# zhenyuw16/Uni3DETR

Hardware: AMD Instinct MI355X
Metric: scenes/sec (fwd+bwd) SUN-RGB-D 20k pts, 300 queries (higher is better)
Workload: dtype bf16

## Files before the change

### include/u3d_hip.h

```cpp
#ifndef U3D_HIP_H_
#define U3D_HIP_H_

#include <stddef.h>
#include <stdint.h>

#ifdef __cplusplus
extern "C" {
#endif

typedef struct ihipStream_t* u3d_stream;

enum {
  U3D_OK = 0,
  U3D_ERR_ARG = -1,
  U3D_ERR_UNSUPPORTED = -2,
  U3D_ERR_LAUNCH = -3,
  U3D_ERR_WORKSPACE = -4
};

enum { U3D_F32 = 0, U3D_BF16 = 1 };

int32_t u3d_version(void);
const char* u3d_strerror(int32_t code);

// ... 194 lines not shown
int32_t u3d_skinny_wgrad_batched(const void* const* dy, const void* const* x, float* const* partial, const int32_t* n, const int32_t* k,
                                 int32_t count, int32_t m, int32_t dy_skinny, u3d_stream s);

int64_t u3d_bn_stats_workspace(int32_t n_cap, int32_t c);
int32_t u3d_bn_stats(const void* x, const int32_t* n_dev, int32_t n_cap, int32_t c, int32_t dtype,
                     double* sums, void* workspace, int64_t workspace_bytes, u3d_stream s);
int32_t u3d_bn_finalize(const double* sums, const int32_t* n_dev, int32_t n_cap, int32_t c, float eps, float momentum,
                        float* running_mean, float* running_var, int64_t* num_batches, float* mean, float* invstd,
                        u3d_stream s);
int32_t u3d_bn_forward_stats(const void* x, const int32_t* n_dev, int32_t n_cap, int32_t c, int32_t dtype, float eps,
                             float momentum, float* running_mean, float* running_var, int64_t* num_batches, float* mean,
                             float* invstd, void* workspace, int64_t workspace_bytes, u3d_stream s);
int32_t u3d_bn_finalize_partials(const double* partial, int32_t nblocks, int32_t rows_per_block, const int32_t* n_dev,
                                 int32_t n_cap, int32_t c, float eps, float momentum, float* running_mean, float* running_var,
                                 int64_t* num_batches, float* mean, float* invstd, u3d_stream s);
int32_t u3d_bn_apply(const void* x, const float* mean, const float* invstd, const float* gamma,
                     const float* beta, const void* residual, int32_t relu, void* y, void* planes,
                     const int32_t* n_dev, int32_t n_cap, int32_t c, int32_t dtype, const int32_t* row_map, const void* post_add,
                     u3d_stream s);
int32_t u3d_bn_bwd_stats(const void* dy, const void* y, const void* x, const float* mean, const float* invstd,
                         const float* gamma, const float* beta, int32_t relu, const int32_t* n_dev, int32_t n_cap,
                         int32_t c, int32_t dtype, double* sums, void* workspace, int64_t workspace_bytes,
                         const int32_t* row_map, float* sums_f32, u3d_stream s);
int32_t u3d_bn_bwd_apply(const void* dy, const void* y, const void* x, const float* mean, const float* invstd,
                         const float* gamma, const float* beta, const double* sums, int32_t relu, void* dx, void* dres, void* planes,
                         const int32_t* n_dev, int32_t n_cap, int32_t c, int32_t dtype, const int32_t* row_map, u3d_stream s);
int32_t u3d_bn_apply_sum(const void* const* x, const float* const* mean, const float* const* invstd, const float* const* gamma,
                         const float* const* beta, const int32_t* const* idx, int32_t levels, void* out, const int32_t* n_dev,
                         int32_t n_cap, int32_t c, int32_t dtype, u3d_stream s);
int32_t u3d_bn_bwd_apply_sum(const void* dout, const void* const* x, const float* const* mean, const float* const* invstd,
                             const float* const* gamma, const float* const* beta, const double* const* sums,
                             const int32_t* const* idx, void* const* dx, int32_t levels, const int32_t* n_dev, int32_t n_cap,
                             int32_t c, int32_t dtype, u3d_stream s);

int32_t u3d_to_dense(const void* feat, const int32_t* coors, const int32_t* n_dev, int32_t n_cap, int32_t c,
                     void* dense, int32_t dz, int32_t dy, int32_t dx, int32_t dtype, u3d_stream s);
int32_t u3d_from_dense(const void* dense, const int32_t* coors, const int32_t* n_dev, int32_t n_cap, int32_t c,
                       void* feat, int32_t dz, int32_t dy, int32_t dx, int32_t dtype, u3d_stream s);

int32_t u3d_gather_rows(const void* in, const int32_t* idx, int32_t n, int32_t row_bytes, void* out, u3d_stream s);
int32_t u3d_scatter_rows(const void* in, const int32_t* idx, int32_t n, int32_t row_bytes, void* out, u3d_stream s);

int32_t u3d_fps(const float* base, const int64_t* set_off, const int32_t* set_n, int32_t nsets, int32_t max_n,
                int32_t m, int32_t* out_idx, float* temp, int64_t temp_stride, int32_t* err, int64_t poll_ticks, int32_t max_wg,
                u3d_stream s);
int32_t u3d_fps2(const float* base, const float* base2, int32_t split, const int64_t* set_off, const int32_t* set_n,
// ... 349 lines not shown
```

### uni3detr_amd/csrc/igemm_wgrad.hip

```cpp
#include "igemm_common.h"
#include "conv_in.h"

#ifndef WGRAD_DMA_SPREAD
#define WGRAD_DMA_SPREAD 1
#endif

template <int WAVES_M, int WAVES_N, int WM, int WN>
__global__ __launch_bounds__(WAVES_M* WAVES_N * 64) void k_igemm_wgrad(const u16* __restrict__ in, const u16* __restrict__ dout,
                                                                        const int* __restrict__ nbr, int ld, float* __restrict__ partial,
                                                                        const int* __restrict__ n_out_dev, int n_out_cap, int cin,
                                                                        int cout, int kvol, int co_blocks) {
  constexpr int NT = WAVES_M * WAVES_N * 64;
  constexpr int TM = WAVES_M * WM * 16, TN = WAVES_N * WN * 16, RK = 64;
  constexpr int LDA = TM + 16, LDD = TN + 16;
  constexpr int A_ELEMS = RK * LDA, D_ELEMS = RK * LDD;
  constexpr int A_SEGS = RK * TM / 8 / NT, D_SEGS = RK * TN / 8 / NT;
  static_assert(RK * TM / 8 % NT == 0 && RK * TN / 8 % NT == 0, "tile/thread mismatch");
  extern __shared__ __attribute__((aligned(16))) u16 smem[];
  constexpr int STAGE_ELEMS = A_ELEMS + D_ELEMS;

  const int n_out = min(*n_out_dev, n_out_cap);
  const int nsplit = gridDim.x, split = blockIdx.x, kap = blockIdx.y;
  const int ci0 = (blockIdx.z / co_blocks) * TM, co0 = (blockIdx.z % co_blocks) * TN;
  const int tid = threadIdx.x, lane = tid & 63, wv = tid >> 6;
// ... 580 lines not shown
    const f32x4 v6 = *(const f32x4*)(p + (long long)(k + 6) * stride), v7 = *(const f32x4*)(p + (long long)(k + 7) * stride);
    a += v0; b += v1; c += v2; d += v3; a += v4; b += v5; c += v6; d += v7;
  }
  for (; k < nsplit; ++k) a += *(const f32x4*)(p + (long long)k * stride);
  return (a + b) + (c + d);
}

struct WgradGroups { unsigned char mult[U3D_WGRAD_BATCH_MAX]; };
__global__ void k_wgrad_batch_reduce(WgradBatch bt, WgradGroups gr, const float* __restrict__ partial, long long n, int nsplit,
                                     long long partial_stride) {
  const int b = blockIdx.y;
  const int g = gr.mult[b];
  long long i = ((long long)blockIdx.x * blockDim.x + threadIdx.x) * 4;
  if (i >= n || g == 0) return;
  *(f32x4*)(bt.dw[b] + i) = wgrad_sum_splits(partial + (long long)b * partial_stride + i, n, nsplit * g);
}

__global__ void k_igemm_wgrad_reduce(const float* __restrict__ partial, float* __restrict__ dw, long long n, int nsplit) {
  long long i = ((long long)blockIdx.x * blockDim.x + threadIdx.x) * 4;
  if (i >= n) return;
  *(f32x4*)(dw + i) = wgrad_sum_splits(partial + i, n, nsplit);
}

__device__ __forceinline__ void wgrad_reduce_tile(const float* __restrict__ partial, long long n, int nsplit, int ca, int cb, int a,
                                                  int b0, int k0, int k1, float (&tile)[64][10]) {
  const int t = threadIdx.x, col = t & 63;
  for (int k = k0 + (t >> 6); k < k1; k += 4) {
    float s = 0.f;
    if (b0 + col < cb) {
      const float* p = partial + ((long long)k * ca + a) * cb + b0 + col;
      float acc[8];
#pragma unroll
      for (int j = 0; j < 8; ++j) acc[j] = 0.f;
      int sp = 0;
      for (; sp + 8 <= nsplit; sp += 8) {
#pragma unroll
        for (int j = 0; j < 8; ++j) acc[j] += p[(long long)(sp + j) * n];
      }
      for (; sp < nsplit; ++sp) acc[0] += p[(long long)sp * n];
      s = ((acc[0] + acc[1]) + (acc[2] + acc[3])) + ((acc[4] + acc[5]) + (acc[6] + acc[7]));
    }
    tile[col][k - k0] = s;
  }
  __syncthreads();
}
__global__ __launch_bounds__(256) void k_igemm_wgrad_reduce_oik(const float* __restrict__ partial, float* __restrict__ dw, long long n,
                                                                int nsplit, int kvol, int cin, int cout) {
  __shared__ float tile[64][10];
  const int ci = blockIdx.x, co0 = blockIdx.y * 64;
  const int kper = (kvol + gridDim.z - 1) / gridDim.z, k0 = blockIdx.z * kper, k1 = min(kvol, k0 + kper);
  wgrad_reduce_tile(partial, n, nsplit, cin, cout, ci, co0, k0, k1, tile);
  const int nk = k1 - k0;
  for (int idx = threadIdx.x; idx < 64 * nk; idx += 256) {
    const int cl = idx / nk, k = idx % nk;
    if (co0 + cl < cout) dw[((long long)(co0 + cl) * cin + ci) * kvol + k0 + k] = tile[cl][k];
  }
}
__global__ __launch_bounds__(256) void k_igemm_wgrad_reduce_abk(const float* __restrict__ partial, float* __restrict__ dw, long long n,
                                                                int nsplit, int kvol, int ca, int cb) {
  __shared__ float tile[64][10];
  const int a = blockIdx.x, b0 = blockIdx.y * 64;
  const int kper = (kvol + gridDim.z - 1) / gridDim.z, k0 = blockIdx.z * kper, k1 = min(kvol, k0 + kper);
  wgrad_reduce_tile(partial, n, nsplit, ca, cb, a, b0, k0, k1, tile);
  const int nk = k1 - k0;
  for (int idx = threadIdx.x; idx < 64 * nk; idx += 256) {
    const int cl = idx / nk, k = idx % nk;
    if (b0 + cl < cb) dw[((long long)a * cb + b0 + cl) * kvol + k0 + k] = tile[cl][k];
  }
}

typedef void (*wgrad_kernel_t)(const u16*, const u16*, const int*, int, float*, const int*, int, int, int, int, int);
typedef void (*wgrad_batch_kernel_t)(WgradBatch, float*, const int*, int, int, int, int, long long);
enum { WG_NONE, WG_CONVIN, WG_NARROW, WG_GLDS8_256, WG_GLDS_256, WG_GLDS_128, WG_GLDS_64, WG_REG_32, WG_REG_16, WG_COUNT };
struct WgradKernel {
  wgrad_kernel_t fn;
  wgrad_batch_kernel_t batch;
  int tile, threads;
  size_t lds;
};
static const WgradKernel WGRAD_KERNELS[WG_COUNT] = {
    {}, {}, {},
    {k_igemm_wgrad_glds8_256, nullptr, 256, 512, 4 * 64 * 256 * 2},
    {k_igemm_wgrad_glds_256, k_wgrad_batch_256, 256, 512, 4 * 64 * 256 * 2},
    {k_igemm_wgrad_glds_128, k_wgrad_batch_128, 128, 256, 4 * 64 * 128 * 2},
    {k_igemm_wgrad_glds_64, k_wgrad_batch_64, 64, 256, 4 * 64 * 64 * 2},
    {k_igemm_wgrad<2, 2, 1, 1>, nullptr, 32, 256, 4 * 64 * (32 + 16) * 2},
    {k_igemm_wgrad<1, 1, 1, 1>, nullptr, 16, 64, 4 * 64 * (16 + 16) * 2},
};
enum WgReduce { WG_RED_OWN, WG_RED_KIO, WG_RED_OIK, WG_RED_ABK };

struct WgradPlan {
// ... 88 lines not shown
  return U3D_OK;
}

static unsigned long long wgrad_lds_mask[WG_COUNT][2] = {};

extern "C" int32_t u3d_igemm_wgrad_bf16(const void* in, const void* dout, const int32_t* nbr, int32_t ld, float* dw,
                                        const int32_t* n_out_dev, int32_t n_out_cap, int32_t cin, int32_t cout, int32_t kvol,
                                        int32_t out_layout, void* workspace, int64_t workspace_bytes, u3d_stream s) {
  U3D_REQUIRE(in && dout && dw && n_out_dev && workspace && (nbr || kvol == 1), U3D_ERR_ARG);
  const WgradPlan p = wgrad_plan(n_out_cap, cin, cout, kvol, nbr != nullptr, out_layout);
  if (!p.served()) return U3D_ERR_UNSUPPORTED;
  if (p.family == WG_NARROW) {
    if (n_out_cap <= 0) { hipMemsetAsync(dw, 0, sizeof(float) * kvol * cin * cout, s); return U3D_OK; }
    return u3d_launch_wgrad_narrow(in, dout, nbr, ld, dw, n_out_dev, n_out_cap, cin, cout, kvol, out_layout, workspace, workspace_bytes, s);
  }
  U3D_REQUIRE(workspace_bytes >= p.workspace, U3D_ERR_WORKSPACE);
  if (p.family == WG_CONVIN) return u3d_launch_conv_in_wgrad(in, dout, nbr, ld, dw, n_out_dev, n_out_cap, kvol, (float*)workspace, s);
  const WgradKernel& k = WGRAD_KERNELS[p.family];
  if (p.lds > 64 * 1024) u3d_allow_lds_impl((const void*)k.fn, (int)p.lds, &wgrad_lds_mask[p.family][0]);
  hipLaunchKernelGGL(k.fn, p.grid, dim3(p.threads), p.lds, s, (const u16*)in, (const u16*)dout, nbr, ld, (float*)workspace, n_out_dev, n_out_cap,
                     cin, cout, kvol, p.co_blocks);
  if (hipGetLastError() != hipSuccess) return U3D_ERR_LAUNCH;
  const long long n = (long long)kvol * cin * cout;
  if (p.reduce == WG_RED_ABK)
    hipLaunchKernelGGL(k_igemm_wgrad_reduce_abk, dim3(cin, u3d_cdiv(cout, 64), kvol > 9 ? 3 : 1), dim3(256), 0, s, (const float*)workspace, dw, n, p.nsplit, kvol, cin, cout);
  else if (p.reduce == WG_RED_OIK)
    hipLaunchKernelGGL(k_igemm_wgrad_reduce_oik, dim3(cin, u3d_cdiv(cout, 64), kvol > 9 ? 3 : 1), dim3(256), 0, s, (const float*)workspace, dw, n, p.nsplit, kvol, cin, cout);
  else
    hipLaunchKernelGGL(k_igemm_wgrad_reduce, dim3(u3d_cdiv(n / 4, 256)), dim3(256), 0, s, (const float*)workspace, dw, n, p.nsplit);
  U3D_CHECK_LAUNCH();
  return U3D_OK;
}

static WgradPlan wgrad_plan_batched(int count, int n_rows, int cin, int cout) {
  const int mn = cin < cout ? cin : cout;
  int tile = (mn >= 256 && cin % 256 == 0 && cout % 256 == 0) ? 256 : ((mn >= 128 && cin % 128 == 0 && cout % 128 == 0) ? 128 : 64);
  const int ntiles = u3d_cdiv(n_rows > 0 ? n_rows : 1, 64);
  WgradPlan p;
  for (;;) {
    p.tile = tile;
    p.ci_blocks = u3d_cdiv(cin, tile);
    p.co_blocks = u3d_cdiv(cout, tile);
    const int per = (count > 0 ? count : 1) * p.ci_blocks * p.co_blocks;
    int ns = u3d_cdiv(768, per);
    int max_ns = ntiles / 8 > 0 ? ntiles / 8 : 1;
    if (ns > max_ns) ns = max_ns;
    if (ns < 1) ns = 1;
    p.nsplit = ns;
    if (tile == 64 || (long long)per * ns >= 192) break;
    tile /= 2;
// ... 34 lines not shown
```

### uni3detr_amd/csrc/rowops.hip

```cpp
#include "common.h"
#include <type_traits>

typedef unsigned short u16;
__device__ __forceinline__ float ld_elem(const float* p, long long i) { return p[i]; }
__device__ __forceinline__ float ld_elem(const u16* p, long long i) { return __uint_as_float(((unsigned)p[i]) << 16); }
__device__ __forceinline__ void st_elem(float* p, long long i, float v) { p[i] = v; }
__device__ __forceinline__ void st_elem(u16* p, long long i, float v) {
  unsigned u = __float_as_uint(v);
  if ((u & 0x7fffffffu) > 0x7f800000u) { p[i] = (u16)((u >> 16) | 0x40u); return; }
  u += 0x7fffu + ((u >> 16) & 1u);
  p[i] = (u16)(u >> 16);
}

static inline int st_rows_per_block(int n_cap, int c) {
  if (n_cap >= 131072) return c >= 128 ? 256 : 512;
  return n_cap >= 32768 ? 128 : 16;
}

template <typename T> struct VecOf;
template <> struct VecOf<float> { static constexpr int N = 4; };
template <> struct VecOf<u16> { static constexpr int N = 8; };

template <typename T>
__device__ __forceinline__ void load_vec(const T* p, float* out);
// ... 8 lines not shown
  unsigned w[4] = {v.x, v.y, v.z, v.w};
#pragma unroll
  for (int i = 0; i < 4; ++i) { out[2 * i] = __uint_as_float(w[i] << 16); out[2 * i + 1] = __uint_as_float(w[i] & 0xffff0000u); }
}

static inline bool al16(const void* p) { return ((uintptr_t)p & 15) == 0; }
template <int V>
__device__ __forceinline__ void load_cols(const float* __restrict__ p, int col0, float* out) {
#pragma unroll
  for (int i = 0; i < V; i += 4) {
    const float4 t = *(const float4*)(p + col0 + i);
    out[i] = t.x; out[i + 1] = t.y; out[i + 2] = t.z; out[i + 3] = t.w;
  }
}
template <int V>
__device__ __forceinline__ void load_cols_d(const double* __restrict__ p, int col0, float scale, float* out) {
#pragma unroll
  for (int i = 0; i < V; i += 2) {
    const double2 t = *(const double2*)(p + col0 + i);
    out[i] = (float)t.x * scale; out[i + 1] = (float)t.y * scale;
  }
}

template <typename T, int MODE>
__global__ __launch_bounds__(256) void k_col_stats_vec(const T* __restrict__ x, const T* __restrict__ dy, const T* __restrict__ y,
                                                       const float* __restrict__ mean, const float* __restrict__ invstd,
                                                       const float* __restrict__ gamma, const float* __restrict__ beta, int relu,
                                                       const int* __restrict__ n_dev, int n_cap, int c, double* __restrict__ partial,
                                                       const int* __restrict__ row_map, int rows_per_block) {
  constexpr int V = VecOf<T>::N;
  extern __shared__ __attribute__((aligned(16))) char smem_raw[];
  double* red = (double*)smem_raw;
  const int n = min(*n_dev, n_cap);
  const int cv = c / V;
  const int cw = cv < 256 ? cv : 256;
  const int rl = 256 / cw;
  const int tcol = threadIdx.x % cw, trow = threadIdx.x / cw;
  const int r0 = blockIdx.x * rows_per_block;
  const int r1 = min(n, r0 + rows_per_block);
  for (int cb = 0; cb < cv; cb += cw) {
    const int vc = cb + tcol;
    float s0[V], s1[V];
#pragma unroll
    for (int e = 0; e < V; ++e) { s0[e] = 0.f; s1[e] = 0.f; }
    const bool active = vc < cv && trow < rl;
    if (active) {
      float mu[V], is[V], ga[V], be[V];
      const bool remask = MODE == 1 && relu && y == nullptr;
      if (MODE == 1) {
        load_cols<V>(mean, vc * V, mu);
        load_cols<V>(invstd, vc * V, is);
        if (remask) { load_cols<V>(gamma, vc * V, ga); load_cols<V>(beta, vc * V, be); }
      }
#pragma unroll 4
      for (int r = r0 + trow; r < r1; r += rl) {
        const long long o = (long long)r * c + (long long)vc * V;
        float xv[V];
        load_vec<T>(x + o, xv);
        if (MODE == 0) {
#pragma unroll
          for (int e = 0; e < V; ++e) { s0[e] += xv[e]; s1[e] += xv[e] * xv[e]; }
        } else {
          float gv[V], yv[V];
          const long long oy = row_map ? (long long)row_map[r] * c + (long long)vc * V : o;
          load_vec<T>(dy + oy, gv);
          if (relu && !remask) load_vec<T>(y + oy, yv);
#pragma unroll
          for (int e = 0; e < V; ++e) {
            float g = gv[e];
            if (remask) yv[e] = (xv[e] - mu[e]) * is[e] * ga[e] + be[e];
            if (relu && !(yv[e] > 0.f)) g = 0.f;
            s0[e] += g;
            s1[e] += g * ((xv[e] - mu[e]) * is[e]);
          }
        }
      }
    }
    const int ncol = cw * V;
    if (trow < rl) {
#pragma unroll
      for (int e = 0; e < V; ++e) {
        red[(0 * rl + trow) * ncol + tcol * V + e] = (double)s0[e];
        red[(1 * rl + trow) * ncol + tcol * V + e] = (double)s1[e];
      }
    }
    __syncthreads();
    const int NP = rl >= 32 ? 8 : 1;
    if (NP > 1) {
      double* red2 = red + 2 * rl * ncol;
      for (int i = threadIdx.x; i < 2 * ncol * NP; i += 256) {
        const int o = i % (2 * ncol), pp = i / (2 * ncol), which = o / ncol, col = o % ncol;
        double a = 0.0;
        for (int j = pp; j < rl; j += NP) a += red[(which * rl + j) * ncol + col];
        red2[pp * 2 * ncol + o] = a;
      }
      __syncthreads();
      for (int i = threadIdx.x; i < 2 * ncol; i += 256) {
        const int which = i / ncol, col = i % ncol;
        if (cb * V + col < c) {
          double a = 0.0;
          for (int pp = 0; pp < NP; ++pp) a += red2[pp * 2 * ncol + i];
          partial[((long long)blockIdx.x * 2 + which) * c + cb * V + col] = a;
        }
      }
    } else {
      for (int i = threadIdx.x; i < 2 * ncol; i += 256) {
        int which = i / ncol, col = i % ncol;
        if (cb * V + col < c) {
          double a = 0.0;
          for (int j = 0; j < rl; ++j) a += red[(which * rl + j) * ncol + col];
          partial[((long long)blockIdx.x * 2 + which) * c + cb * V + col] = a;
        }
      }
    }
    __syncthreads();
  }
}

template <typename T, int MODE>
__global__ __launch_bounds__(256) void k_col_stats(const T* __restrict__ x, const T* __restrict__ dy, const T* __restrict__ y,
                                                   const float* __restrict__ mean, const float* __restrict__ invstd,
                                                   const float* __restrict__ gamma, const float* __restrict__ beta, int relu,
                                                   const int* __restrict__ n_dev, int n_cap, int c, double* __restrict__ partial,
                                                   int rows_per_block) {
  __shared__ double red[2][256];
  const int n = min(*n_dev, n_cap);
  const int cw = c < 256 ? c : 256;
  const int rl = 256 / cw;
  const int tcol = threadIdx.x % cw, trow = threadIdx.x / cw;
  const int r0 = blockIdx.x * rows_per_block;
  const int r1 = min(n, r0 + rows_per_block);
  for (int cb = 0; cb < c; cb += cw) {
    int col = cb + tcol;
    double s0 = 0.0, s1 = 0.0;
    if (col < c && trow < rl) {
      float mu = 0.f, is = 0.f, ga = 0.f, be = 0.f;
      const bool remask = MODE == 1 && relu && y == nullptr;
      if (MODE == 1) { mu = mean[col]; is = invstd[col]; }
      if (remask) { ga = gamma[col]; be = beta[col]; }
// ... 27 lines not shown
}

#define FIN_THREADS 1024
#define FIN_LANES (FIN_THREADS / 16)
__device__ __forceinline__ void fin_reduce(const double* __restrict__ partial, int used, int c, int col0, double (*red)[16]) {
  const int v = threadIdx.x & 15, bl = threadIdx.x >> 4;
  const int which = v >> 3, col = col0 + (v & 7);
  double a = 0.0;
  if (col < c) {
#pragma unroll 8
    for (int b = bl; b < used; b += FIN_LANES) a += partial[((long long)b * 2 + which) * c + col];
  }
  red[bl][v] = a;
  __syncthreads();
  if (threadIdx.x < 16) {
    double s0 = 0.0, s1 = 0.0, s2 = 0.0, s3 = 0.0;
#pragma unroll 4
    for (int j = 0; j < FIN_LANES; j += 4) { s0 += red[j][threadIdx.x]; s1 += red[j + 1][threadIdx.x]; s2 += red[j + 2][threadIdx.x]; s3 += red[j + 3][threadIdx.x]; }
    red[0][threadIdx.x] = (s0 + s1) + (s2 + s3);
  }
  __syncthreads();
}

__global__ __launch_bounds__(FIN_THREADS) void k_col_stats_final(const double* __restrict__ partial, int nblocks, const int* __restrict__ n_dev,
                                                                 int n_cap, int c, double* __restrict__ sums, float* __restrict__ sums_f32,
                                                                 int rows_per_block) {
  __shared__ double red[FIN_LANES][16];
  const int n = min(*n_dev, n_cap);
  int used = rows_per_block > 0 ? (n + rows_per_block - 1) / rows_per_block : nblocks;
  if (used > nblocks) used = nblocks;
  const int col0 = blockIdx.x * 8;
  fin_reduce(partial, used, c, col0, red);
  if (threadIdx.x < 16) {
    const int which = threadIdx.x >> 3, col = col0 + (threadIdx.x & 7);
    if (col < c) {
      const double s = red[0][threadIdx.x];
      sums[which * c + col] = s;
      if (sums_f32) sums_f32[which * c + col] = (float)s;
    }
  }
}

extern "C" int64_t u3d_bn_stats_workspace(int32_t n_cap, int32_t c) {
  return (int64_t)u3d_cdiv(n_cap > 0 ? n_cap : 1, st_rows_per_block(n_cap, c)) * 2 * c * 8;
}

template <int MODE>
static int run_stats(const void* x, const void* dy, const void* y, const float* mean, const float* invstd, const float* gamma,
                     const float* beta, int relu, const int32_t* n_dev, int n_cap, int c, int dtype, double* sums, void* ws, int64_t ws_bytes, hipStream_t s,
                     const int32_t* row_map = nullptr, float* sums_f32 = nullptr) {
  U3D_REQUIRE(x && n_dev && sums && ws && c > 0, U3D_ERR_ARG);
  U3D_REQUIRE(!row_map || (dtype == U3D_F32 ? c % 4 == 0 : c % 8 == 0), U3D_ERR_UNSUPPORTED);
  if (n_cap <= 0) { hipMemsetAsync(sums, 0, sizeof(double) * 2 * c, s); return U3D_OK; }
  U3D_REQUIRE(ws_bytes >= u3d_bn_stats_workspace(n_cap, c), U3D_ERR_WORKSPACE);
  const int rpb = st_rows_per_block(n_cap, c);
  int nb = u3d_cdiv(n_cap, rpb);
  const bool pal = al16(mean) && al16(invstd) && al16(gamma) && al16(beta);
  U3D_REQUIRE(!row_map || pal, U3D_ERR_ARG);
  if (dtype == U3D_F32) {
    if (c % 4 == 0 && pal) {
      int cw = (c / 4) < 256 ? (c / 4) : 256; int rl = 256 / cw;
      size_t lds = (size_t)2 * (rl + (rl >= 32 ? 8 : 0)) * cw * 4 * sizeof(double);
      hipLaunchKernelGGL((k_col_stats_vec<float, MODE>), dim3(nb), dim3(256), lds, s, (const float*)x, (const float*)dy, (const float*)y, mean, invstd, gamma, beta, relu, n_dev, n_cap, c, (double*)ws, row_map, rpb);
    } else {
      hipLaunchKernelGGL((k_col_stats<float, MODE>), dim3(nb), dim3(256), 0, s, (const float*)x, (const float*)dy, (const float*)y, mean, invstd, gamma, beta, relu, n_dev, n_cap, c, (double*)ws, rpb);
    }
  } else if (dtype == U3D_BF16) {
    if (c % 8 == 0 && pal) {
      int cw = (c / 8) < 256 ? (c / 8) : 256; int rl = 256 / cw;
      size_t lds = (size_t)2 * (rl + (rl >= 32 ? 8 : 0)) * cw * 8 * sizeof(double);
      hipLaunchKernelGGL((k_col_stats_vec<u16, MODE>), dim3(nb), dim3(256), lds, s, (const u16*)x, (const u16*)dy, (const u16*)y, mean, invstd, gamma, beta, relu, n_dev, n_cap, c, (double*)ws, row_map, rpb);
    } else {
      hipLaunchKernelGGL((k_col_stats<u16, MODE>), dim3(nb), dim3(256), 0, s, (const u16*)x, (const u16*)dy, (const u16*)y, mean, invstd, gamma, beta, relu, n_dev, n_cap, c, (double*)ws, rpb);
    }
  } else return U3D_ERR_UNSUPPORTED;
  hipLaunchKernelGGL(k_col_stats_final, dim3(u3d_cdiv(c, 8)), dim3(FIN_THREADS), 0, s, (const double*)ws, nb, n_dev, n_cap, c, sums, sums_f32, rpb);
  U3D_CHECK_LAUNCH();
  return U3D_OK;
}

extern "C" int32_t u3d_bn_stats(const void* x, const int32_t* n_dev, int32_t n_cap, int32_t c, int32_t dtype, double* sums,
                                void* workspace, int64_t workspace_bytes, u3d_stream s) {
  return run_stats<0>(x, nullptr, nullptr, nullptr, nullptr, nullptr, nullptr, 0, n_dev, n_cap, c, dtype, sums, workspace, workspace_bytes, s);
}
extern "C" int32_t u3d_bn_bwd_stats(const void* dy, const void* y, const void* x, const float* mean, const float* invstd,
                                    const float* gamma, const float* beta, int32_t relu, const int32_t* n_dev, int32_t n_cap,
                                    int32_t c, int32_t dtype, double* sums, void* workspace, int64_t workspace_bytes,
                                    const int32_t* row_map, float* sums_f32, u3d_stream s) {
  U3D_REQUIRE(dy && mean && invstd && (!relu || y || (gamma && beta)), U3D_ERR_ARG);
  return run_stats<1>(x, dy, y, mean, invstd, gamma, beta, relu, n_dev, n_cap, c, dtype, sums, workspace, workspace_bytes, s, row_map, sums_f32);
}

#define CS_ROWS 32
template <typename T, int V>
__global__ __launch_bounds__(256) void k_colsum_partial(const T* __restrict__ x, int n, int c, float* __restrict__ partial) {
  __shared__ float red[256 * 8];
  const int cv = (c + V - 1) / V;
  const int cw = cv < 256 ? cv : 256;
  const int rl = 256 / cw;
  const int tcol = threadIdx.x % cw, trow = threadIdx.x / cw;
  const int r0 = blockIdx.x * CS_ROWS, r1 = min(n, r0 + CS_ROWS);
  for (int cb = 0; cb < cv; cb += cw) {
    const int vc = cb + tcol;
    float s[V];
#pragma unroll
    for (int e = 0; e < V; ++e) s[e] = 0.f;
    if (vc < cv && trow < rl) {
      for (int r = r0 + trow; r < r1; r += rl) {
        const long long o = (long long)r * c + (long long)vc * V;
        float xv[V];
        if constexpr (V == 1) xv[0] = ld_elem(x, o); else load_vec<T>(x + o, xv);
#pragma unroll
        for (int e = 0; e < V; ++e) s[e] += xv[e];
// ... 971 lines not shown
```

### uni3detr_amd/native.py

```python
import collections
import ctypes as C
import os

import numpy as np
import torch

from . import abi

_HERE = os.path.dirname(os.path.abspath(__file__))
LIB_PATH = os.environ.get("U3D_LIB_PATH") or os.path.join(_HERE, "libu3d_hip.so")

_ABI = abi.load()
_K = _ABI.constants


def _struct(c_name, py_name):
    return abi.structure(_ABI.structs[c_name], py_name)


def _slot_names(prefix):
    names = sorted((v, n[len(prefix):]) for n, v in _K.items() if n.startswith(prefix))
    assert [v for v, _ in names] == list(range(len(names))) and names[-1][1] == "COUNT" and _K[prefix + "COUNT"] == len(names) - 1
    return [n for _, n in names[:-1]]

# ... 966 lines not shown
    return (sums, s32) if want_f32 else sums


def bn_bwd_apply(dy, y, x, mean, invstd, gamma, sums, relu, n_dev, want_dres, beta=None, row_map=None, want_planes=False):
    n, c = x.shape
    dx = torch.empty_like(x)
    dres = torch.empty_like(x) if want_dres else None
    planes = torch.empty((2 * n, c), dtype=torch.bfloat16, device=x.device) if want_planes and x.dtype == torch.float32 else None
    for planes in (planes, None):
        rc = lib().u3d_bn_bwd_apply(_ptr(dy), _ptr(y), _ptr(x), _ptr(mean), _ptr(invstd), _ptr(gamma), _ptr(beta), _ptr(sums), int(relu),
                                    _ptr(dx), _ptr(dres), _ptr(planes), _ptr(n_dev), n, c, dtype_code(x), _ptr(row_map), _stream())
        if planes is None or rc != U3D_ERR_UNSUPPORTED:
            break
    _check(rc, "bn_bwd_apply")
    return (dx, dres, planes) if want_planes else (dx, dres)


def _opt_ptr_array(tensors):
    arr = (C.c_void_p * len(tensors))()
    for i, t in enumerate(tensors):
        assert t is None or (t.is_cuda and t.is_contiguous()), "device-contiguous tensor required"
        arr[i] = None if t is None else t.data_ptr()
    return arr


def bn_apply_sum(xs, means, invstds, gammas, betas, idxs, n_dev):
    n, c = xs[0].shape
    assert all(x.shape == (n, c) and x.dtype == xs[0].dtype for x in xs)
    out = torch.empty_like(xs[0])
    rc = lib().u3d_bn_apply_sum(_opt_ptr_array(xs), _opt_ptr_array(means), _opt_ptr_array(invstds), _opt_ptr_array(gammas),
                                _opt_ptr_array(betas), _opt_ptr_array(idxs), len(xs), _ptr(out), _ptr(n_dev), n, c, dtype_code(xs[0]),
                                _stream())
    if rc == U3D_ERR_UNSUPPORTED:
        return None
    _check(rc, "bn_apply_sum")
    return out


def bn_bwd_apply_sum(dout, xs, means, invstds, gammas, betas, sums, idxs, n_dev):
    n, c = dout.shape
    dxs = [torch.empty_like(x) for x in xs]
    _check(lib().u3d_bn_bwd_apply_sum(_ptr(dout), _opt_ptr_array(xs), _opt_ptr_array(means), _opt_ptr_array(invstds),
                                      _opt_ptr_array(gammas), _opt_ptr_array(betas), _opt_ptr_array(sums), _opt_ptr_array(idxs),
                                      _opt_ptr_array(dxs), len(xs), _ptr(n_dev), n, c, dtype_code(dout), _stream()), "bn_bwd_apply_sum")
    return dxs

# ... 1206 lines not shown
```

### uni3detr_amd/sparse.py

```python
import collections
import contextlib
import os

import torch

from . import native as nv
from .shadow import conv_weights, halo_packs

K3, S1, P1 = (3, 3, 3), (1, 1, 1), (1, 1, 1)


class Level:

    def __init__(self, grid, coords, n, n_dev):
        self.grid, self.coords, self.n, self.n_dev = grid, coords, n, n_dev
        self.dims, self.batch = grid.dims, grid.batch
        self._subm = None
        self._halo = None

    def halo(self):
        if self._halo is None:
            h = nv.SubmHalo(self.subm_tables()[0], self.n_dev, self.n) if self.n <= nv.SubmHalo.MAX_ROWS else None
            self._halo = h if (h is not None and h.ok) else False
        return self._halo or None
# ... 598 lines not shown
            if stats is not None:
                mean, invstd = nv.bn_finalize_partials(stats, tile_rows, n_dev, n, bn.eps, mom, bn.running_mean, bn.running_var,
                                                       bn.num_batches_tracked)
            else:
                mean, invstd = nv.bn_forward_stats(x, n_dev, bn.eps, mom, bn.running_mean, bn.running_var, bn.num_batches_tracked)
            means.append(mean)
            invstds.append(invstd)
        g32, b32 = [g.float() for g in gammas], [b.float() for b in betas]
        idxs = [s[3] for s in specs]
        out = nv.bn_apply_sum(xs, means, invstds, g32, b32, idxs, n_dev)
        if out is None:
            raise nv.U3DError("bn_apply_sum refused a shape bn_rows_sum_serves() let through")
        ctx.save_for_backward(*xs, *means, *invstds, *g32, *b32)
        ctx.n_dev, ctx.idxs, ctx.invs = n_dev, idxs, [s[4] for s in specs]
        ctx.pdtypes = [g.dtype for g in gammas]
        return out

    @staticmethod
    def backward(ctx, dout):
        L = len(ctx.idxs)
        t = ctx.saved_tensors
        xs, means, invstds, gammas, betas = (t[i * L:(i + 1) * L] for i in range(5))
        dout = dout.contiguous()
        stats = [nv.bn_bwd_stats(dout, None, xs[i], means[i], invstds[i], True, ctx.n_dev, gammas[i], betas[i], ctx.invs[i], want_f32=True)
                 for i in range(L)]
        dxs = nv.bn_bwd_apply_sum(dout, xs, means, invstds, gammas, betas, [s[0] for s in stats], ctx.idxs, ctx.n_dev)
        grads = []
        for i in range(L):
            s32 = stats[i][1] if ctx.pdtypes[i] == torch.float32 else stats[i][1].to(ctx.pdtypes[i])
            grads += [dxs[i], s32[1], s32[0]]
        return (None, None, *grads)


def bn_rows_sum(xs, bns, n_dev, stats, idxs, invs):
    specs = [(bn, None if st is None else st[0], 0 if st is None else st[1], idx, inv) for bn, st, idx, inv in zip(bns, stats, idxs, invs)]
    flat = [t for x, bn in zip(xs, bns) for t in (x, bn.weight, bn.bias)]
    return _BNRowsSum.apply(n_dev, specs, *flat)


class _ToDense(torch.autograd.Function):
    @staticmethod
    def forward(ctx, feats, lvl):
        ctx.lvl = lvl
        vol = nv.to_dense(feats, lvl.coords, lvl.n_dev, lvl.batch, lvl.dims)
        ctx.active = _ACTIVE[0] = None
        if ACTIVE_FIRST_CONV and ctx.needs_input_grad[0] and feats.dtype == torch.bfloat16 and feats.is_cuda:
            ctx.set_materialize_grads(False)
            ctx.active = _ACTIVE[0] = ActiveInput(lvl, feats, vol)
# ... 48 lines not shown
```

Baseline: 441.9.

## Vectorize wgrad split-reduce and batch BN backward stats across levels

```diff
diff --git a/include/u3d_hip.h b/include/u3d_hip.h
--- a/include/u3d_hip.h
+++ b/include/u3d_hip.h
@@ -240,6 +240,11 @@
                          const float* gamma, const float* beta, int32_t relu, const int32_t* n_dev, int32_t n_cap,
                          int32_t c, int32_t dtype, double* sums, void* workspace, int64_t workspace_bytes,
                          const int32_t* row_map, float* sums_f32, u3d_stream s);
+int32_t u3d_bn_bwd_stats_levels(const void* const* dy, const void* const* y, const void* const* x, const float* const* mean,
+                                const float* const* invstd, const float* const* gamma, const float* const* beta, int32_t relu,
+                                const int32_t* const* row_map, int32_t levels, const int32_t* n_dev, int32_t n_cap, int32_t c,
+                                int32_t dtype, double* const* sums, float* const* sums_f32, void* workspace, int64_t workspace_bytes,
+                                u3d_stream s);
 int32_t u3d_bn_bwd_apply(const void* dy, const void* y, const void* x, const float* mean, const float* invstd,
                          const float* gamma, const float* beta, const double* sums, int32_t relu, void* dx, void* dres, void* planes,
                          const int32_t* n_dev, int32_t n_cap, int32_t c, int32_t dtype, const int32_t* row_map, u3d_stream s);
diff --git a/uni3detr_amd/csrc/col_stats_vec_body.inc b/uni3detr_amd/csrc/col_stats_vec_body.inc
--- /dev/null
+++ b/uni3detr_amd/csrc/col_stats_vec_body.inc
@@ -0,0 +1,87 @@
+  constexpr int V = VecOf<T>::N;
+  extern __shared__ __attribute__((aligned(16))) char smem_raw[];
+  double* red = (double*)smem_raw;
+  const int n = min(*n_dev, n_cap);
+  const int cv = c / V;
+  const int cw = cv < 256 ? cv : 256;
+  const int rl = 256 / cw;
+  const int tcol = threadIdx.x % cw, trow = threadIdx.x / cw;
+  const int r0 = blockIdx.x * rows_per_block;
+  const int r1 = min(n, r0 + rows_per_block);
+  for (int cb = 0; cb < cv; cb += cw) {
+    const int vc = cb + tcol;
+    float s0[V], s1[V];
+#pragma unroll
+    for (int e = 0; e < V; ++e) { s0[e] = 0.f; s1[e] = 0.f; }
+    const bool active = vc < cv && trow < rl;
+    if (active) {
+      float mu[V], is[V], ga[V], be[V];
+      const bool remask = MODE == 1 && relu && y == nullptr;
+      if (MODE == 1) {
+        load_cols<V>(mean, vc * V, mu);
+        load_cols<V>(invstd, vc * V, is);
+        if (remask) { load_cols<V>(gamma, vc * V, ga); load_cols<V>(beta, vc * V, be); }
+      }
+#pragma unroll 4
+      for (int r = r0 + trow; r < r1; r += rl) {
+        const long long o = (long long)r * c + (long long)vc * V;
+        float xv[V];
+        load_vec<T>(x + o, xv);
+        if (MODE == 0) {
+#pragma unroll
+          for (int e = 0; e < V; ++e) { s0[e] += xv[e]; s1[e] += xv[e] * xv[e]; }
+        } else {
+          float gv[V], yv[V];
+          const long long oy = row_map ? (long long)row_map[r] * c + (long long)vc * V : o;
+          load_vec<T>(dy + oy, gv);
+          if (relu && !remask) load_vec<T>(y + oy, yv);
+#pragma unroll
+          for (int e = 0; e < V; ++e) {
+            float g = gv[e];
+            if (remask) yv[e] = (xv[e] - mu[e]) * is[e] * ga[e] + be[e];
+            if (relu && !(yv[e] > 0.f)) g = 0.f;
+            s0[e] += g;
+            s1[e] += g * ((xv[e] - mu[e]) * is[e]);
+          }
+        }
+      }
+    }
+    const int ncol = cw * V;
+    if (trow < rl) {
+#pragma unroll
+      for (int e = 0; e < V; ++e) {
+        red[(0 * rl + trow) * ncol + tcol * V + e] = (double)s0[e];
+        red[(1 * rl + trow) * ncol + tcol * V + e] = (double)s1[e];
+      }
+    }
+    __syncthreads();
+    const int NP = rl >= 32 ? 8 : 1;
+    if (NP > 1) {
+      double* red2 = red + 2 * rl * ncol;
+      for (int i = threadIdx.x; i < 2 * ncol * NP; i += 256) {
+        const int o = i % (2 * ncol), pp = i / (2 * ncol), which = o / ncol, col = o % ncol;
+        double a = 0.0;
+        for (int j = pp; j < rl; j += NP) a += red[(which * rl + j) * ncol + col];
+        red2[pp * 2 * ncol + o] = a;
+      }
+      __syncthreads();
+      for (int i = threadIdx.x; i < 2 * ncol; i += 256) {
+        const int which = i / ncol, col = i % ncol;
+        if (cb * V + col < c) {
+          double a = 0.0;
+          for (int pp = 0; pp < NP; ++pp) a += red2[pp * 2 * ncol + i];
+          partial[((long long)blockIdx.x * 2 + which) * c + cb * V + col] = a;
+        }
+      }
+    } else {
+      for (int i = threadIdx.x; i < 2 * ncol; i += 256) {
+        int which = i / ncol, col = i % ncol;
+        if (cb * V + col < c) {
+          double a = 0.0;
+          for (int j = 0; j < rl; ++j) a += red[(which * rl + j) * ncol + col];
+          partial[((long long)blockIdx.x * 2 + which) * c + cb * V + col] = a;
+        }
+      }
+    }
+    __syncthreads();
+  }
diff --git a/uni3detr_amd/csrc/igemm_wgrad.hip b/uni3detr_amd/csrc/igemm_wgrad.hip
--- a/uni3detr_amd/csrc/igemm_wgrad.hip
+++ b/uni3detr_amd/csrc/igemm_wgrad.hip
@@ -626,51 +626,81 @@
   *(f32x4*)(dw + i) = wgrad_sum_splits(partial + i, n, nsplit);
 }
 
-__device__ __forceinline__ void wgrad_reduce_tile(const float* __restrict__ partial, long long n, int nsplit, int ca, int cb, int a,
-                                                  int b0, int k0, int k1, float (&tile)[64][10]) {
-  const int t = threadIdx.x, col = t & 63;
-  for (int k = k0 + (t >> 6); k < k1; k += 4) {
-    float s = 0.f;
-    if (b0 + col < cb) {
-      const float* p = partial + ((long long)k * ca + a) * cb + b0 + col;
-      float acc[8];
-#pragma unroll
-      for (int j = 0; j < 8; ++j) acc[j] = 0.f;
+#ifndef WGRAD_REDUCE_MIN_WGS
+#define WGRAD_REDUCE_MIN_WGS 1024
+#endif
+static inline int wgrad_reduce_ashift(int kvol, int ca, int cb) {
+  int sh = kvol > 18 ? 1 : (kvol > 9 ? 2 : (kvol > 4 ? 3 : 4));
+  while (sh > 0 && (ca % (1 << sh) != 0 || (long long)(ca >> sh) * u3d_cdiv(cb, 64) < WGRAD_REDUCE_MIN_WGS)) --sh;
+  return sh;
+}
+static inline size_t wgrad_reduce_lds(bool abk, int kvol, int ashift) {
+  return sizeof(float) * (abk ? (size_t)(64 * kvol + 1) << ashift : (size_t)64 * ((kvol << ashift) + 1));
+}
+template <bool ABK>
+__device__ __forceinline__ void wgrad_reduce_block(const float* __restrict__ partial, float* __restrict__ dw, long long n, int nsplit,
+                                                   int kvol, int ca, int cb, int ashift) {
+  extern __shared__ __attribute__((aligned(16))) float wr_tile[];
+  const int ablk = 1 << ashift, a0 = blockIdx.x << ashift, b0 = blockIdx.y * 64;
+  const int pitch = ABK ? 64 * kvol + 1 : ablk * kvol + 1;
+  const int items = (kvol << ashift) * 16;
+  for (int i = threadIdx.x; i < items; i += 256) {
+    const int c4 = i & 15, row = i >> 4, al = row & (ablk - 1), k = row >> ashift;
+    f32x4 s = (f32x4){0.f, 0.f, 0.f, 0.f};
+    if (a0 + al < ca && b0 + c4 * 4 < cb) {
+      const float* p = partial + ((long long)k * ca + a0 + al) * cb + b0 + c4 * 4;
+      f32x4 acc[8];
+#pragma unroll
+      for (int j = 0; j < 8; ++j) acc[j] = s;
       int sp = 0;
+#pragma unroll 2
       for (; sp + 8 <= nsplit; sp += 8) {
-#pragma unroll
-        for (int j = 0; j < 8; ++j) acc[j] += p[(long long)(sp + j) * n];
-      }
-      for (; sp < nsplit; ++sp) acc[0] += p[(long long)sp * n];
+        f32x4 v[8];
+#pragma unroll
+        for (int j = 0; j < 8; ++j) v[j] = *(const f32x4*)(p + (long long)(sp + j) * n);
+#pragma unroll
+        for (int j = 0; j < 8; ++j) acc[j] += v[j];
+      }
+      {
+        f32x4 v[7];
+        const int rem = nsplit - sp;
+#pragma unroll
+        for (int j = 0; j < 7; ++j)
+          if (j < rem) v[j] = *(const f32x4*)(p + (long long)(sp + j) * n);
+#pragma unroll
+        for (int j = 0; j < 7; ++j)
+          if (j < rem) acc[0] += v[j];
+      }
       s = ((acc[0] + acc[1]) + (acc[2] + acc[3])) + ((acc[4] + acc[5]) + (acc[6] + acc[7]));
     }
-    tile[col][k - k0] = s;
+#pragma unroll
+    for (int e = 0; e < 4; ++e) {
+      const int cl = c4 * 4 + e;
+      wr_tile[ABK ? al * pitch + cl * kvol + k : cl * pitch + al * kvol + k] = s[e];
+    }
   }
   __syncthreads();
+  if (ABK) {
+    const int run = min(64, cb - b0) * kvol;
+    for (int al = 0; al < ablk && a0 + al < ca; ++al) {
+      float* __restrict__ o = dw + ((long long)(a0 + al) * cb + b0) * kvol;
+      for (int j = threadIdx.x; j < run; j += 256) o[j] = wr_tile[al * pitch + j];
+    }
+  } else {
+    const int run = min(ablk, ca - a0) * kvol, ncl = min(64, cb - b0);
+    for (int idx = threadIdx.x; idx < ncl * run; idx += 256) {
+      const int cl = idx / run, j = idx - cl * run;
+      dw[((long long)(b0 + cl) * ca + a0) * kvol + j] = wr_tile[cl * pitch + j];
+    }
+  }
 }
 __global__ __launch_bounds__(256) void k_igemm_wgrad_reduce_oik(const float* __restrict__ partial, float* __restrict__ dw, long long n,
-                                                                int nsplit, int kvol, int cin, int cout) {
-  __shared__ float tile[64][10];
-  const int ci = blockIdx.x, co0 = blockIdx.y * 64;
-  const int kper = (kvol + gridDim.z - 1) / gridDim.z, k0 = blockIdx.z * kper, k1 = min(kvol, k0 + kper);
-  wgrad_reduce_tile(partial, n, nsplit, cin, cout, ci, co0, k0, k1, tile);
-  const int nk = k1 - k0;
-  for (int idx = threadIdx.x; idx < 64 * nk; idx += 256) {
-    const int cl = idx / nk, k = idx % nk;
-    if (co0 + cl < cout) dw[((long long)(co0 + cl) * cin + ci) * kvol + k0 + k] = tile[cl][k];
-  }
+                                                                int nsplit, int kvol, int cin, int cout, int ashift) {
+  wgrad_reduce_block<false>(partial, dw, n, nsplit, kvol, cin, cout, ashift);
 }
 __global__ __launch_bounds__(256) void k_igemm_wgrad_reduce_abk(const float* __restrict__ partial, float* __restrict__ dw, long long n,
-                                                                int nsplit, int kvol, int ca, int cb) {
-  __shared__ float tile[64][10];
-  const int a = blockIdx.x, b0 = blockIdx.y * 64;
-  const int kper = (kvol + gridDim.z - 1) / gridDim.z, k0 = blockIdx.z * kper, k1 = min(kvol, k0 + kper);
-  wgrad_reduce_tile(partial, n, nsplit, ca, cb, a, b0, k0, k1, tile);
-  const int nk = k1 - k0;
-  for (int idx = threadIdx.x; idx < 64 * nk; idx += 256) {
-    const int cl = idx / nk, k = idx % nk;
-    if (b0 + cl < cb) dw[((long long)a * cb + b0 + cl) * kvol + k0 + k] = tile[cl][k];
-  }
+                                                                int nsplit, int kvol, int ca, int cb, int ashift) {
+  wgrad_reduce_block<true>(partial, dw, n, nsplit, kvol, ca, cb, ashift);
 }
 
 typedef void (*wgrad_kernel_t)(const u16*, const u16*, const int*, int, float*, const int*, int, int, int, int, int);
@@ -805,10 +835,13 @@
                      cin, cout, kvol, p.co_blocks);
   if (hipGetLastError() != hipSuccess) return U3D_ERR_LAUNCH;
   const long long n = (long long)kvol * cin * cout;
-  if (p.reduce == WG_RED_ABK)
-    hipLaunchKernelGGL(k_igemm_wgrad_reduce_abk, dim3(cin, u3d_cdiv(cout, 64), kvol > 9 ? 3 : 1), dim3(256), 0, s, (const float*)workspace, dw, n, p.nsplit, kvol, cin, cout);
-  else if (p.reduce == WG_RED_OIK)
-    hipLaunchKernelGGL(k_igemm_wgrad_reduce_oik, dim3(cin, u3d_cdiv(cout, 64), kvol > 9 ? 3 : 1), dim3(256), 0, s, (const float*)workspace, dw, n, p.nsplit, kvol, cin, cout);
+  if (p.reduce == WG_RED_ABK || p.reduce == WG_RED_OIK) {
+    const bool abk = p.reduce == WG_RED_ABK;
+    const int sh = wgrad_reduce_ashift(kvol, cin, cout);
+    const dim3 grid(u3d_cdiv(cin, 1 << sh), u3d_cdiv(cout, 64));
+    if (abk) hipLaunchKernelGGL(k_igemm_wgrad_reduce_abk, grid, dim3(256), wgrad_reduce_lds(true, kvol, sh), s, (const float*)workspace, dw, n, p.nsplit, kvol, cin, cout, sh);
+    else hipLaunchKernelGGL(k_igemm_wgrad_reduce_oik, grid, dim3(256), wgrad_reduce_lds(false, kvol, sh), s, (const float*)workspace, dw, n, p.nsplit, kvol, cin, cout, sh);
+  }
   else
     hipLaunchKernelGGL(k_igemm_wgrad_reduce, dim3(u3d_cdiv(n / 4, 256)), dim3(256), 0, s, (const float*)workspace, dw, n, p.nsplit);
   U3D_CHECK_LAUNCH();
diff --git a/uni3detr_amd/csrc/rowops.hip b/uni3detr_amd/csrc/rowops.hip
--- a/uni3detr_amd/csrc/rowops.hip
+++ b/uni3detr_amd/csrc/rowops.hip
@@ -54,99 +54,42 @@
   }
 }
 
+static inline size_t st_vec_lds(int c, int v) {
+  const int cw = (c / v) < 256 ? (c / v) : 256, rl = 256 / cw;
+  return (size_t)2 * (rl + (rl >= 32 ? 8 : 0)) * cw * v * sizeof(double);
+}
 template <typename T, int MODE>
 __global__ __launch_bounds__(256) void k_col_stats_vec(const T* __restrict__ x, const T* __restrict__ dy, const T* __restrict__ y,
                                                        const float* __restrict__ mean, const float* __restrict__ invstd,
                                                        const float* __restrict__ gamma, const float* __restrict__ beta, int relu,
                                                        const int* __restrict__ n_dev, int n_cap, int c, double* __restrict__ partial,
                                                        const int* __restrict__ row_map, int rows_per_block) {
-  constexpr int V = VecOf<T>::N;
-  extern __shared__ __attribute__((aligned(16))) char smem_raw[];
-  double* red = (double*)smem_raw;
-  const int n = min(*n_dev, n_cap);
-  const int cv = c / V;
-  const int cw = cv < 256 ? cv : 256;
-  const int rl = 256 / cw;
-  const int tcol = threadIdx.x % cw, trow = threadIdx.x / cw;
-  const int r0 = blockIdx.x * rows_per_block;
-  const int r1 = min(n, r0 + rows_per_block);
-  for (int cb = 0; cb < cv; cb += cw) {
-    const int vc = cb + tcol;
-    float s0[V], s1[V];
-#pragma unroll
-    for (int e = 0; e < V; ++e) { s0[e] = 0.f; s1[e] = 0.f; }
-    const bool active = vc < cv && trow < rl;
-    if (active) {
-      float mu[V], is[V], ga[V], be[V];
-      const bool remask = MODE == 1 && relu && y == nullptr;
-      if (MODE == 1) {
-        load_cols<V>(mean, vc * V, mu);
-        load_cols<V>(invstd, vc * V, is);
-        if (remask) { load_cols<V>(gamma, vc * V, ga); load_cols<V>(beta, vc * V, be); }
-      }
-#pragma unroll 4
-      for (int r = r0 + trow; r < r1; r += rl) {
-        const long long o = (long long)r * c + (long long)vc * V;
-        float xv[V];
-        load_vec<T>(x + o, xv);
-        if (MODE == 0) {
-#pragma unroll
-          for (int e = 0; e < V; ++e) { s0[e] += xv[e]; s1[e] += xv[e] * xv[e]; }
-        } else {
-          float gv[V], yv[V];
-          const long long oy = row_map ? (long long)row_map[r] * c + (long long)vc * V : o;
-          load_vec<T>(dy + oy, gv);
-          if (relu && !remask) load_vec<T>(y + oy, yv);
-#pragma unroll
-          for (int e = 0; e < V; ++e) {
-            float g = gv[e];
-            if (remask) yv[e] = (xv[e] - mu[e]) * is[e] * ga[e] + be[e];
-            if (relu && !(yv[e] > 0.f)) g = 0.f;
-            s0[e] += g;
-            s1[e] += g * ((xv[e] - mu[e]) * is[e]);
-          }
-        }
-      }
-    }
-    const int ncol = cw * V;
-    if (trow < rl) {
-#pragma unroll
-      for (int e = 0; e < V; ++e) {
-        red[(0 * rl + trow) * ncol + tcol * V + e] = (double)s0[e];
-        red[(1 * rl + trow) * ncol + tcol * V + e] = (double)s1[e];
-      }
-    }
-    __syncthreads();
-    const int NP = rl >= 32 ? 8 : 1;
-    if (NP > 1) {
-      double* red2 = red + 2 * rl * ncol;
-      for (int i = threadIdx.x; i < 2 * ncol * NP; i += 256) {
-        const int o = i % (2 * ncol), pp = i / (2 * ncol), which = o / ncol, col = o % ncol;
-        double a = 0.0;
-        for (int j = pp; j < rl; j += NP) a += red[(which * rl + j) * ncol + col];
-        red2[pp * 2 * ncol + o] = a;
-      }
-      __syncthreads();
-      for (int i = threadIdx.x; i < 2 * ncol; i += 256) {
-        const int which = i / ncol, col = i % ncol;
-        if (cb * V + col < c) {
-          double a = 0.0;
-          for (int pp = 0; pp < NP; ++pp) a += red2[pp * 2 * ncol + i];
-          partial[((long long)blockIdx.x * 2 + which) * c + cb * V + col] = a;
-        }
-      }
-    } else {
-      for (int i = threadIdx.x; i < 2 * ncol; i += 256) {
-        int which = i / ncol, col = i % ncol;
-        if (cb * V + col < c) {
-          double a = 0.0;
-          for (int j = 0; j < rl; ++j) a += red[(which * rl + j) * ncol + col];
-          partial[((long long)blockIdx.x * 2 + which) * c + cb * V + col] = a;
-        }
-      }
-    }
-    __syncthreads();
-  }
+#include "col_stats_vec_body.inc"
+}
+#define ST_MAX_LEVELS 4
+struct StatsLevels {
+  const void *x[ST_MAX_LEVELS], *dy[ST_MAX_LEVELS], *y[ST_MAX_LEVELS];
+  const float *mean[ST_MAX_LEVELS], *invstd[ST_MAX_LEVELS], *gamma[ST_MAX_LEVELS], *beta[ST_MAX_LEVELS];
+  const int* row_map[ST_MAX_LEVELS];
+  double* sums[ST_MAX_LEVELS];
+  float* sums_f32[ST_MAX_LEVELS];
+};
+template <typename T>
+__global__ __launch_bounds__(256) void k_col_stats_vec_levels(StatsLevels lv, int relu, const int* __restrict__ n_dev, int n_cap, int c,
+                                                              double* __restrict__ levels_partial, long long level_stride,
+                                                              int rows_per_block) {
+  constexpr int MODE = 1;
+  const int l = blockIdx.y;
+  const T* __restrict__ x = (const T*)lv.x[l];
+  const T* __restrict__ dy = (const T*)lv.dy[l];
+  const T* __restrict__ y = (const T*)lv.y[l];
+  const float* __restrict__ mean = lv.mean[l];
+  const float* __restrict__ invstd = lv.invstd[l];
+  const float* __restrict__ gamma = lv.gamma[l];
+  const float* __restrict__ beta = lv.beta[l];
+  const int* __restrict__ row_map = lv.row_map[l];
+  double* __restrict__ partial = levels_partial + l * level_stride;
+#include "col_stats_vec_body.inc"
 }
 
 template <typename T, int MODE>
@@ -220,9 +163,9 @@
   __syncthreads();
 }
 
-__global__ __launch_bounds__(FIN_THREADS) void k_col_stats_final(const double* __restrict__ partial, int nblocks, const int* __restrict__ n_dev,
-                                                                 int n_cap, int c, double* __restrict__ sums, float* __restrict__ sums_f32,
-                                                                 int rows_per_block) {
+__device__ __forceinline__ void col_stats_final_block(const double* __restrict__ partial, int nblocks, const int* __restrict__ n_dev,
+                                                      int n_cap, int c, double* __restrict__ sums, float* __restrict__ sums_f32,
+                                                      int rows_per_block) {
   __shared__ double red[FIN_LANES][16];
   const int n = min(*n_dev, n_cap);
   int used = rows_per_block > 0 ? (n + rows_per_block - 1) / rows_per_block : nblocks;
@@ -237,6 +180,17 @@
       if (sums_f32) sums_f32[which * c + col] = (float)s;
     }
   }
+}
+__global__ __launch_bounds__(FIN_THREADS) void k_col_stats_final(const double* __restrict__ partial, int nblocks, const int* __restrict__ n_dev,
+                                                                 int n_cap, int c, double* __restrict__ sums, float* __restrict__ sums_f32,
+                                                                 int rows_per_block) {
+  col_stats_final_block(partial, nblocks, n_dev, n_cap, c, sums, sums_f32, rows_per_block);
+}
+__global__ __launch_bounds__(FIN_THREADS) void k_col_stats_final_levels(StatsLevels lv, const double* __restrict__ partial, long long level_stride,
+                                                                        int nblocks, const int* __restrict__ n_dev, int n_cap, int c,
+                                                                        int rows_per_block) {
+  const int l = blockIdx.y;
+  col_stats_final_block(partial + l * level_stride, nblocks, n_dev, n_cap, c, lv.sums[l], lv.sums_f32[l], rows_per_block);
 }
 
 extern "C" int64_t u3d_bn_stats_workspace(int32_t n_cap, int32_t c) {
@@ -257,16 +211,14 @@
   U3D_REQUIRE(!row_map || pal, U3D_ERR_ARG);
   if (dtype == U3D_F32) {
     if (c % 4 == 0 && pal) {
-      int cw = (c / 4) < 256 ? (c / 4) : 256; int rl = 256 / cw;
-      size_t lds = (size_t)2 * (rl + (rl >= 32 ? 8 : 0)) * cw * 4 * sizeof(double);
+      const size_t lds = st_vec_lds(c, 4);
       hipLaunchKernelGGL((k_col_stats_vec<float, MODE>), dim3(nb), dim3(256), lds, s, (const float*)x, (const float*)dy, (const float*)y, mean, invstd, gamma, beta, relu, n_dev, n_cap, c, (double*)ws, row_map, rpb);
     } else {
       hipLaunchKernelGGL((k_col_stats<float, MODE>), dim3(nb), dim3(256), 0, s, (const float*)x, (const float*)dy, (const float*)y, mean, invstd, gamma, beta, relu, n_dev, n_cap, c, (double*)ws, rpb);
     }
   } else if (dtype == U3D_BF16) {
     if (c % 8 == 0 && pal) {
-      int cw = (c / 8) < 256 ? (c / 8) : 256; int rl = 256 / cw;
-      size_t lds = (size_t)2 * (rl + (rl >= 32 ? 8 : 0)) * cw * 8 * sizeof(double);
+      const size_t lds = st_vec_lds(c, 8);
       hipLaunchKernelGGL((k_col_stats_vec<u16, MODE>), dim3(nb), dim3(256), lds, s, (const u16*)x, (const u16*)dy, (const u16*)y, mean, invstd, gamma, beta, relu, n_dev, n_cap, c, (double*)ws, row_map, rpb);
     } else {
       hipLaunchKernelGGL((k_col_stats<u16, MODE>), dim3(nb), dim3(256), 0, s, (const u16*)x, (const u16*)dy, (const u16*)y, mean, invstd, gamma, beta, relu, n_dev, n_cap, c, (double*)ws, rpb);
@@ -287,6 +239,39 @@
                                     const int32_t* row_map, float* sums_f32, u3d_stream s) {
   U3D_REQUIRE(dy && mean && invstd && (!relu || y || (gamma && beta)), U3D_ERR_ARG);
   return run_stats<1>(x, dy, y, mean, invstd, gamma, beta, relu, n_dev, n_cap, c, dtype, sums, workspace, workspace_bytes, s, row_map, sums_f32);
+}
+extern "C" int32_t u3d_bn_bwd_stats_levels(const void* const* dy, const void* const* y, const void* const* x, const float* const* mean,
+                                           const float* const* invstd, const float* const* gamma, const float* const* beta,
+                                           int32_t relu, const int32_t* const* row_map, int32_t levels, const int32_t* n_dev,
+                                           int32_t n_cap, int32_t c, int32_t dtype, double* const* sums, float* const* sums_f32,
+                                           void* workspace, int64_t workspace_bytes, u3d_stream s) {
+  U3D_REQUIRE(dy && y && x && mean && invstd && gamma && beta && row_map && sums && sums_f32 && n_dev && workspace && c > 0 &&
+              levels >= 1 && levels <= ST_MAX_LEVELS, U3D_ERR_ARG);
+  const int v = dtype == U3D_F32 ? 4 : 8;
+  if ((dtype != U3D_F32 && dtype != U3D_BF16) || c % v != 0) return U3D_ERR_UNSUPPORTED;
+  StatsLevels lv = {};
+  for (int l = 0; l < levels; ++l) {
+    U3D_REQUIRE(dy[l] && x[l] && mean[l] && invstd[l] && sums[l] && (!relu || y[l] || (gamma[l] && beta[l])), U3D_ERR_ARG);
+    if (!(al16(mean[l]) && al16(invstd[l]) && al16(gamma[l]) && al16(beta[l]))) return U3D_ERR_UNSUPPORTED;
+    lv.x[l] = x[l]; lv.dy[l] = dy[l]; lv.y[l] = y[l]; lv.mean[l] = mean[l]; lv.invstd[l] = invstd[l]; lv.gamma[l] = gamma[l];
+    lv.beta[l] = beta[l]; lv.row_map[l] = row_map[l]; lv.sums[l] = sums[l]; lv.sums_f32[l] = sums_f32[l];
+  }
+  if (n_cap <= 0) {
+    for (int l = 0; l < levels; ++l) hipMemsetAsync(sums[l], 0, sizeof(double) * 2 * c, s);
+    return U3D_OK;
+  }
+  const int64_t level_bytes = u3d_bn_stats_workspace(n_cap, c);
+  U3D_REQUIRE(workspace_bytes >= level_bytes * levels, U3D_ERR_WORKSPACE);
+  const int rpb = st_rows_per_block(n_cap, c), nb = u3d_cdiv(n_cap, rpb);
+  const long long stride = level_bytes / (long long)sizeof(double);
+  const size_t lds = st_vec_lds(c, v);
+  if (dtype == U3D_F32)
+    hipLaunchKernelGGL(k_col_stats_vec_levels<float>, dim3(nb, levels), dim3(256), lds, s, lv, relu, n_dev, n_cap, c, (double*)workspace, stride, rpb);
+  else
+    hipLaunchKernelGGL(k_col_stats_vec_levels<u16>, dim3(nb, levels), dim3(256), lds, s, lv, relu, n_dev, n_cap, c, (double*)workspace, stride, rpb);
+  hipLaunchKernelGGL(k_col_stats_final_levels, dim3(u3d_cdiv(c, 8), levels), dim3(FIN_THREADS), 0, s, lv, (const double*)workspace, stride, nb, n_dev, n_cap, c, rpb);
+  U3D_CHECK_LAUNCH();
+  return U3D_OK;
 }
 
 #define CS_ROWS 32
diff --git a/uni3detr_amd/native.py b/uni3detr_amd/native.py
--- a/uni3detr_amd/native.py
+++ b/uni3detr_amd/native.py
@@ -1012,6 +1012,26 @@
         assert t is None or (t.is_cuda and t.is_contiguous()), "device-contiguous tensor required"
         arr[i] = None if t is None else t.data_ptr()
     return arr
+
+
+def bn_bwd_stats_levels(dys, ys, xs, means, invstds, relu, n_dev, gammas, betas, row_maps, ws=None):
+    n, c = xs[0].shape
+    L = len(xs)
+    assert all(x.shape == (n, c) and x.dtype == xs[0].dtype for x in xs)
+    sums = torch.empty((L, 2, c), dtype=torch.float64, device=xs[0].device)
+    s32 = torch.empty((L, 2, c), dtype=torch.float32, device=xs[0].device)
+    wsb = int(lib().u3d_bn_stats_workspace(n, c)) * L
+    if ws is None:
+        ws = torch.empty(wsb, dtype=torch.uint8, device=xs[0].device)
+    rc = lib().u3d_bn_bwd_stats_levels(_opt_ptr_array(dys), _opt_ptr_array(ys), _opt_ptr_array(xs), _opt_ptr_array(means),
+                                       _opt_ptr_array(invstds), _opt_ptr_array(gammas), _opt_ptr_array(betas), int(relu),
+                                       _opt_ptr_array(row_maps), L, _ptr(n_dev), n, c, dtype_code(xs[0]), _opt_ptr_array(list(sums)),
+                                       _opt_ptr_array(list(s32)), _ptr(ws), ws.numel(), _stream())
+    if rc == U3D_ERR_UNSUPPORTED:
+        return [bn_bwd_stats(dys[i], ys[i], xs[i], means[i], invstds[i], relu, n_dev, gammas[i], betas[i], row_maps[i], want_f32=True)
+                for i in range(L)]
+    _check(rc, "bn_bwd_stats_levels")
+    return [(sums[i], s32[i]) for i in range(L)]
 
 
 def bn_apply_sum(xs, means, invstds, gammas, betas, idxs, n_dev):
diff --git a/uni3detr_amd/sparse.py b/uni3detr_amd/sparse.py
--- a/uni3detr_amd/sparse.py
+++ b/uni3detr_amd/sparse.py
@@ -644,8 +644,7 @@
         t = ctx.saved_tensors
         xs, means, invstds, gammas, betas = (t[i * L:(i + 1) * L] for i in range(5))
         dout = dout.contiguous()
-        stats = [nv.bn_bwd_stats(dout, None, xs[i], means[i], invstds[i], True, ctx.n_dev, gammas[i], betas[i], ctx.invs[i], want_f32=True)
-                 for i in range(L)]
+        stats = nv.bn_bwd_stats_levels([dout] * L, [None] * L, xs, means, invstds, True, ctx.n_dev, gammas, betas, ctx.invs)
         dxs = nv.bn_bwd_apply_sum(dout, xs, means, invstds, gammas, betas, [s[0] for s in stats], ctx.idxs, ctx.n_dev)
         grads = []
         for i in range(L):
```

Result: no change. 444.0 (median of 6 runs) (+0.5%).
